# vasil-pashov/sparse_matrix_math

Measured on AMD Instinct MI355X. Metric: CSR SpMV GB/s (% HBM peak) + BiCGStab iters/sec, 10M rows, 1/2/4/8 GPU, higher is better.
Workload: dtype f32

## Files before the change

include/smm_hip.h:

```cpp
#ifndef SMM_HIP_H
#define SMM_HIP_H

#include <stddef.h>

#ifdef __cplusplus
extern "C" {
#endif

#define SMM_HIP_VERSION_MAJOR 0
#define SMM_HIP_VERSION_MINOR 1

#define SMM_HIP_OK 0
#define SMM_HIP_ERR_INVALID (-1)
#define SMM_HIP_ERR_HIP (-2)
#define SMM_HIP_ERR_NO_DEVICE (-3)
#define SMM_HIP_ERR_PRECOND (-4)
#define SMM_HIP_ERR_NOMEM (-5)
#define SMM_HIP_ERR_COMM (-6)

#define SMM_SOLVER_SUCCESS 0
#define SMM_SOLVER_DIVERGED 1
#define SMM_SOLVER_MAX_ITERATIONS_REACHED 2

#define SMM_OP_ASSIGN 0
// ... 22 lines not shown
#define SMM_PATTERN_CONST 3

typedef struct smm_hip_csr smm_hip_csr;
typedef struct smm_hip_precond smm_hip_precond;
typedef void* smm_hip_stream;

int smm_hip_init(int device);
int smm_hip_shutdown(void);
const char* smm_hip_last_error(void);
int smm_hip_uses_std_fma(void);
int smm_hip_device_info(char* name, size_t name_cap, int* cus, size_t* hbm_bytes);
int smm_hip_stream_synchronize(smm_hip_stream stream);

int smm_hip_debug_fail_next_alloc(size_t min_bytes);
int smm_hip_profile_enable(int on);
int smm_hip_profile_read(double* spmv_ms, long long* spmv_launches, int reset);
int smm_hip_profile_read_waits(double* exposed_ms, long long* pairs, int reset);

int smm_hip_csr_create_f32(int rows, int cols, const int* start, const int* positions, const float* values, smm_hip_csr** out);
int smm_hip_csr_create_f64(int rows, int cols, const int* start, const int* positions, const double* values, smm_hip_csr** out);
int smm_hip_csr_create_dev_f32(int rows, int cols, const int* d_start, const int* d_positions, const float* d_values, smm_hip_csr** out);
int smm_hip_csr_create_dev_f64(int rows, int cols, const int* d_start, const int* d_positions, const double* d_values, smm_hip_csr** out);
int smm_hip_csr_destroy(smm_hip_csr* m);
int smm_hip_csr_info(const smm_hip_csr* m, int* rows, int* cols, int* nnz, int* dtype, int* first_active_start);
int smm_hip_csr_set_kernel(smm_hip_csr* m, int family, int lanes_per_row);
int smm_hip_csr_get_kernel(const smm_hip_csr* m, int* family, int* lanes_per_row);
int smm_hip_csr_tile_info(const smm_hip_csr* m, int* tiles, int* tile_nnz_cap, int* tile_max_rows, int* tile_kernel);
int smm_hip_csr_pattern_info(const smm_hip_csr* m, int* encoding, int* offsets);
int smm_hip_csr_kernel_desc(const smm_hip_csr* m, char* name, int name_cap, long long* bytes_per_launch);
int smm_hip_set_march_min_rows(long long const_diagonals_rows, long long values_read_rows);
int smm_hip_set_cg_lazy_x_min_bytes(long long bytes);
int smm_hip_set_cg_fuse_p(int on);
int smm_hip_csr_pattern_allow_const(smm_hip_csr* m, int allow);
int smm_hip_csr_autotune(smm_hip_csr* m);

#define SMM_UPDATE_SET 0
#define SMM_UPDATE_ADD 1
int smm_hip_csr_scale_f32(smm_hip_csr* m, float alpha, smm_hip_stream stream);
int smm_hip_csr_scale_f64(smm_hip_csr* m, double alpha, smm_hip_stream stream);
int smm_hip_csr_axpy_f32(smm_hip_csr* m, float alpha, const smm_hip_csr* other, smm_hip_stream stream);
int smm_hip_csr_axpy_f64(smm_hip_csr* m, double alpha, const smm_hip_csr* other, smm_hip_stream stream);
int smm_hip_csr_zero_f32(smm_hip_csr* m, smm_hip_stream stream);
int smm_hip_csr_zero_f64(smm_hip_csr* m, smm_hip_stream stream);
int smm_hip_csr_update_entries_f32(smm_hip_csr* m, int n, const int* rows, const int* cols, const float* values, int mode, unsigned char* found);
int smm_hip_csr_update_entries_f64(smm_hip_csr* m, int n, const int* rows, const int* cols, const double* values, int mode, unsigned char* found);
int smm_hip_csr_update_entries_dev_f32(smm_hip_csr* m, int n, const int* d_rows, const int* d_cols, const float* d_values, int mode, unsigned char* d_found,
                                       smm_hip_stream stream);
int smm_hip_csr_update_entries_dev_f64(smm_hip_csr* m, int n, const int* d_rows, const int* d_cols, const double* d_values, int mode, unsigned char* d_found,
                                       smm_hip_stream stream);
int smm_hip_csr_set_values_f32(smm_hip_csr* m, const float* values);
int smm_hip_csr_set_values_f64(smm_hip_csr* m, const double* values);
int smm_hip_csr_set_values_dev_f32(smm_hip_csr* m, const float* d_values, smm_hip_stream stream);
int smm_hip_csr_set_values_dev_f64(smm_hip_csr* m, const double* d_values, smm_hip_stream stream);
int smm_hip_csr_get_values_f32(const smm_hip_csr* m, float* values);
int smm_hip_csr_get_values_f64(const smm_hip_csr* m, double* values);
int smm_hip_csr_values_changed_f32(smm_hip_csr* m, smm_hip_stream stream);
int smm_hip_csr_values_changed_f64(smm_hip_csr* m, smm_hip_stream stream);
int smm_hip_csr_same_pattern(const smm_hip_csr* a, const smm_hip_csr* b, int* same);

int smm_hip_spmv_f32(const smm_hip_csr* m, int op, const float* lhs, const float* x, float* out);
int smm_hip_spmv_f64(const smm_hip_csr* m, int op, const double* lhs, const double* x, double* out);
int smm_hip_spmv_dev_f32(const smm_hip_csr* m, int op, const float* d_lhs, const float* d_x, float* d_out, smm_hip_stream stream);
int smm_hip_spmv_dev_f64(const smm_hip_csr* m, int op, const double* d_lhs, const double* d_x, double* d_out, smm_hip_stream stream);

int smm_hip_dot_f32(int n, const float* a, const float* b, float* result);
int smm_hip_dot_f64(int n, const double* a, const double* b, double* result);
// ... 177 lines not shown
```

sparse_matrix_math_amd/_lib.py:

```python
import ctypes
import os
from ctypes import POINTER, c_char_p, c_double, c_float, c_int, c_longlong, c_size_t, c_ulonglong, c_void_p

_HERE = os.path.dirname(os.path.abspath(__file__))

SMM_HIP_OK = 0
SMM_HIP_ERR_INVALID = -1
SMM_HIP_ERR_HIP = -2
SMM_HIP_ERR_NO_DEVICE = -3
SMM_HIP_ERR_PRECOND = -4
SMM_HIP_ERR_NOMEM = -5
SMM_HIP_ERR_COMM = -6


class SmmHipError(RuntimeError):
    def __init__(self, code, message):
        super().__init__(f"libsmm_hip error {code}: {message}")
        self.code = code


def library_path(fma=False):
    if os.environ.get("SMM_HIP_LIBRARY"):
        return os.environ["SMM_HIP_LIBRARY"]
    name = "libsmm_hip_fma.so" if fma else "libsmm_hip.so"
# ... 45 lines not shown
    "smm_hip_csr_update_entries": (c_int, [_P, c_int, _P, _P, _P, c_int, _P]),
    "smm_hip_csr_update_entries_dev": (c_int, [_P, c_int, _P, _P, _P, c_int, _P, _P]),
    "smm_hip_csr_set_values": (c_int, [_P, _P]),
    "smm_hip_csr_set_values_dev": (c_int, [_P, _P, _P]),
    "smm_hip_csr_get_values": (c_int, [_P, _P]),
    "smm_hip_csr_values_changed": (c_int, [_P, _P]),
}



_PLAIN = {
    "smm_hip_init": (c_int, [c_int]),
    "smm_hip_shutdown": (c_int, []),
    "smm_hip_last_error": (c_char_p, []),
    "smm_hip_uses_std_fma": (c_int, []),
    "smm_hip_device_info": (c_int, [c_char_p, c_size_t, POINTER(c_int), POINTER(c_size_t)]),
    "smm_hip_stream_synchronize": (c_int, [_P]),
    "smm_hip_debug_fail_next_alloc": (c_int, [c_size_t]),
    "smm_hip_profile_enable": (c_int, [c_int]),
    "smm_hip_profile_read": (c_int, [POINTER(c_double), POINTER(c_longlong), c_int]),
    "smm_hip_profile_read_waits": (c_int, [POINTER(c_double), POINTER(c_longlong), c_int]),
    "smm_hip_csr_destroy": (c_int, [_P]),
    "smm_hip_csr_info": (c_int, [_P, POINTER(c_int), POINTER(c_int), POINTER(c_int), POINTER(c_int), POINTER(c_int)]),
    "smm_hip_csr_set_kernel": (c_int, [_P, c_int, c_int]),
    "smm_hip_csr_get_kernel": (c_int, [_P, POINTER(c_int), POINTER(c_int)]),
    "smm_hip_csr_autotune": (c_int, [_P]),
    "smm_hip_csr_tile_info": (c_int, [_P, POINTER(c_int), POINTER(c_int), POINTER(c_int), POINTER(c_int)]),
    "smm_hip_csr_pattern_info": (c_int, [_P, POINTER(c_int), POINTER(c_int)]),
    "smm_hip_csr_kernel_desc": (c_int, [_P, c_char_p, c_int, POINTER(c_longlong)]),
    "smm_hip_set_march_min_rows": (c_int, [c_longlong, c_longlong]),
    "smm_hip_set_cg_lazy_x_min_bytes": (c_int, [c_longlong]),
    "smm_hip_set_cg_fuse_p": (c_int, [c_int]),
    "smm_hip_csr_pattern_allow_const": (c_int, [_P, c_int]),
    "smm_hip_csr_same_pattern": (c_int, [_P, _P, POINTER(c_int)]),
    "smm_hip_precond_create": (c_int, [_P, c_int, POINTER(_P)]),
    "smm_hip_precond_create_block": (c_int, [_P, c_int, c_int, POINTER(_P)]),
    "smm_hip_precond_create_block_capped": (c_int, [_P, c_int, c_int, c_int, POINTER(_P)]),
    "smm_hip_precond_block_level_cap": (c_int, [_P, POINTER(c_int)]),
    "smm_hip_precond_create_block_ex": (c_int, [_P, c_int, c_int, c_int, c_int, POINTER(_P)]),
    "smm_hip_precond_block_rows": (c_int, [_P, _P, c_size_t, _P]),
    "smm_hip_precond_block_record_bytes": (c_int, [_P, POINTER(c_int), POINTER(c_int), POINTER(c_int)]),
    "smm_hip_precond_block_count": (c_int, [_P, POINTER(c_int)]),
    "smm_hip_precond_block_bounds": (c_int, [_P, _P, c_size_t]),
    "smm_hip_precond_destroy": (c_int, [_P]),
    "smm_hip_precond_set_sweep": (c_int, [_P, c_int]),
    "smm_hip_precond_take_error": (c_int, [_P, _P]),
    "smm_hip_precond_info": (c_int, [_P, POINTER(c_int), POINTER(c_int), POINTER(c_int)]),
    "smm_hip_gen_poisson2d_nnz": (c_longlong, [c_int, c_int]),
    "smm_hip_gen_stencil3d_nnz": (c_longlong, [c_int, c_int, c_int]),
    "smm_hip_gen_banded_nnz": (c_longlong, [c_int, c_int, c_ulonglong, c_int]),
    "smm_hip_gen_banded_row_start": (c_longlong, [c_int, c_int, c_ulonglong, c_int, c_int]),
    "smm_hip_partials_count": (c_int, []),
    "smm_hip_finish_len": (c_int, []),
    "smm_hip_finish_totals_offset": (c_int, []),
    "smm_hip_cg_resident": (c_int, [c_int]),
    "smm_hip_bicgstab_resident": (c_int, [c_int]),
    "smm_hip_bicgstab_ws_destroy": (c_int, [_P]),
    "smm_hip_cg_ws_status": (c_int, [_P, _P, POINTER(c_int)]),
    "smm_hip_bicgstab_ws_bind": (c_int, [_P, _P, _P, _P]),
    "smm_hip_bicgstab_ws_pointers": (c_int, [_P, POINTER(_P), POINTER(_P), POINTER(_P), POINTER(_P), POINTER(_P), POINTER(_P)]),
    "smm_hip_comm_unique_id": (c_int, [_P]),
    "smm_hip_comm_create_rccl": (c_int, [c_int, c_int, _P, POINTER(_P)]),
    "smm_hip_comm_create_host": (c_int, [c_int, c_int, HOST_ALLREDUCE_FN, HOST_SENDRECV_FN, _P, POINTER(_P)]),
    "smm_hip_comm_create_self": (c_int, [POINTER(_P)]),
    "smm_hip_comm_destroy": (c_int, [_P]),
    "smm_hip_comm_info": (c_int, [_P, POINTER(c_int), POINTER(c_int), POINTER(c_int)]),
# ... 86 lines not shown
```

sparse_matrix_math_amd/csrc/smm_csr_update.hip:

```cpp
#include <algorithm>
#include <cstring>

#include <rocprim/device/device_radix_sort.hpp>

#include "smm_internal.h"

namespace smm {
namespace {

constexpr int UTPB = 256;

typedef float upd_f32x4 __attribute__((ext_vector_type(4)));
typedef double upd_f64x2 __attribute__((ext_vector_type(2)));
template <typename T>
struct Vec16;
template <>
struct Vec16<float> {
	using type = upd_f32x4;
};
template <>
struct Vec16<double> {
	using type = upd_f64x2;
};

// ... 240 lines not shown
}

bool isConstForm(const smm_hip_csr* m) {
	return m->pat_state.load(std::memory_order_acquire) == 1 && m->pat_encoding == 0 && m->pat_const && m->d_pat_cval &&
	       static_cast<int>(m->pat_cval_host.size()) == m->pat_k;
}

template <typename T>
int valuesEdited(smm_hip_csr* m, hipStream_t s, int edit, T alpha, const smm_hip_csr* other) {
	if (m->pat_state.load(std::memory_order_acquire) != 1 || m->pat_encoding != 0) return SMM_HIP_OK;
	std::lock_guard<std::mutex> lock(m->tileMutex);
	if (isConstForm(m)) {
		const int k = m->pat_k;
		std::vector<unsigned long long> bits(m->pat_cval_host);
		bool exact = true;
		if (edit == EDIT_SCALE) {
			for (int j = 0; j < k; ++j) bits[j] = toBits<T>(fromBits<T>(bits[j]) * alpha);
		} else if (edit == EDIT_ZERO) {
			for (int j = 0; j < k; ++j) bits[j] = 0;
		} else if (edit == EDIT_AXPY && other && isConstForm(other) && other->pat_k == k && other->pat_offs_host == m->pat_offs_host) {
			for (int j = 0; j < k; ++j) bits[j] = toBits<T>(fromBits<T>(bits[j]) + alpha * fromBits<T>(other->pat_cval_host[j]));
		} else {
			exact = false;
		}
		if (exact) {
			cvalUpdateKernel<T><<<1, CMAX, 0, s>>>(k, edit == EDIT_SCALE ? 0 : edit == EDIT_AXPY ? 1 : 2, alpha, m->d_pat_cval,
			                                       edit == EDIT_AXPY ? other->d_pat_cval : nullptr);
			SMM_HIP_TRY(hipGetLastError());
			m->pat_cval_host = bits;
		} else {
			SMM_TRY(reverifyConst(m, s));
		}
	}
	return refreshResEll(m, s);
}

int checkHandle(const smm_hip_csr* m, int dtype, const char* what) {
	if (!m) {
		setError("%s: null matrix", what);
		return SMM_HIP_ERR_INVALID;
	}
	if (m->dtype != dtype) {
		setError("%s: the matrix holds the other element type", what);
		return SMM_HIP_ERR_INVALID;
	}
	return ensureInit();
}

template <typename T>
int scaleDev(smm_hip_csr* m, T alpha, hipStream_t s) {
	SMM_TRY(checkHandle(m, dtypeOf<T>(), "csr_scale"));
	SMM_TRY(ensureCsrReady(m, s, true));
	if (m->nnz > 0) {
		T* v = static_cast<T*>(m->d_values);
		if (reinterpret_cast<uintptr_t>(v) % 16 == 0) valuesUpdateKernel<T, false, true><<<gridFor(m->nnz / (16 / sizeof(T)) + 1), UTPB, 0, s>>>(m->nnz, alpha, v, nullptr);
		else valuesUpdateKernel<T, false, false><<<gridFor(m->nnz), UTPB, 0, s>>>(m->nnz, alpha, v, nullptr);
		SMM_HIP_TRY(hipGetLastError());
	}
	return valuesEdited<T>(m, s, EDIT_SCALE, alpha, nullptr);
}

template <typename T>
int axpyDev(smm_hip_csr* m, T alpha, const smm_hip_csr* other, hipStream_t s) {
	SMM_TRY(checkHandle(m, dtypeOf<T>(), "csr_axpy"));
	SMM_TRY(checkHandle(other, dtypeOf<T>(), "csr_axpy"));
	bool same = false;
// ... 180 lines not shown
```

sparse_matrix_math_amd/csrc/smm_internal.h:

```cpp
#pragma once
#include <hip/hip_runtime.h>

#include <cstddef>
#include <cstdint>
#include <cstdio>
#include <atomic>
#include <chrono>
#include <cstdlib>
#include <cstring>
#include <mutex>
#include <string>
#include <type_traits>
#include <vector>

#include "../../include/smm_hip.h"

namespace smm {

void setError(const char* fmt, ...);
int hipFail(hipError_t e, const char* what, const char* file, int line);

#define SMM_HIP_TRY(expr)                                             \
	do {                                                              \
		hipError_t _e = (expr);                                       \
// ... 87 lines not shown
}

struct smm_hip_csr {
	int rows = 0, cols = 0, nnz = 0, dtype = 0;
	int firstActiveStart = 0;
	bool ready = false;
	bool kernelForced = false;
	std::mutex readyMutex;
	int* d_start = nullptr;
	int* d_positions = nullptr;
	void* d_values = nullptr;
	bool owns = false;
	std::atomic<int> kernelWord{SMM_SPMV_VECTOR | (4 << 8)};
	int family() const { return kernelWord.load(std::memory_order_acquire) & 0xFF; }
	int lanes() const { return kernelWord.load(std::memory_order_acquire) >> 8; }
	void setKernel(int family, int lanes) { kernelWord.store((family & 0xFF) | (lanes << 8), std::memory_order_release); }
	std::mutex adoptMutex;
	int* d_rowblocks = nullptr;
	int n_rowblocks = 0;
	int stream_nnz_cap = 0;
	int stream_max_rows = 0;
	int stream_chunk_tiles = 0;
	int stream_mid_len = 0;
	int max_row_len = -1;
	std::mutex tileMutex;
	std::atomic<int> pat_state{0};
	int pat_encoding = 0;
	unsigned short* d_pat_codes = nullptr;
	bool pat_const = false;
	unsigned long long* d_pat_cval = nullptr;
	std::vector<unsigned long long> pat_cval_host;
	void* d_res_ell = nullptr;
	bool pat_const_off = false;
	int pat_max_off = 0;
	bool march_ok = false;
	int march_P = 0, march_H = 0, march_lo = 0, march_hi = 0;
	bool march_clusters = false;
	unsigned* d_pat_masks32 = nullptr;
	unsigned char* d_pat_masks8 = nullptr;
	std::vector<int> pat_offs_host;
	int pat_k = 0;
	int* d_pat_off = nullptr;
	unsigned long long* d_pat_masks = nullptr;
	int* d_pat_rowblocks = nullptr;
	int pat_n_rowblocks = 0;
	int pat_nnz_cap = 0;
	int pat_max_rows = 0;
	int pat_chunk_tiles = 0;
	int split_tile_max[3] = {-1, -1, -1};
	bool split_uneven = false;
	std::atomic<unsigned long long> uid{0};
	std::mutex editMutex;
	std::vector<std::pair<unsigned long long, bool>> patternSeen;
};

struct smm_hip_precond {
	int kind = SMM_PRECOND_NONE;
	int dtype = 0;
	const smm_hip_csr* a = nullptr;
	void* d_values = nullptr;
	size_t n_values = 0;
	int* d_order_lo = nullptr;
	int* d_order_up = nullptr;
	std::vector<int> lvl_ptr_lo, lvl_ptr_up;
	struct smm_precond_plan* plan = nullptr;
	struct smm_precond_block* blk = nullptr;
// ... 16 lines not shown
constexpr int SPMV_FINISH = 0x200;
constexpr int SPMV_LEAVE_ROOM = 0x400;
constexpr int SPMV_DIV_LHS = 0x800;
constexpr int SPMV_OP_DIV = 3;
constexpr int SPMV_ADD_DIV = 0x1000;
constexpr int SPMV_OP_ADD_DIV = 4;
constexpr int SPMV_HALF_TILES = 0x2000;
constexpr int SPMV_NO_FULL_ROWS = 0x4000;
constexpr int PARTS_TOTALS = 2 * NPART;
constexpr int PARTS_TICKETS = 16;
constexpr int PARTS_LEN = 2 * NPART + 2 + 2 * (PARTS_TICKETS + 1);
template <typename T>
__host__ __device__ inline unsigned* partsTicket(T* partials) { return reinterpret_cast<unsigned*>(partials + PARTS_TOTALS + 2); }
inline int spmvOutFlags(const smm_hip_csr* m, size_t elemBytes) {
	static const int forced = [] {
		const char* env = getenv("SMM_HIP_NT_OUT");
		return env ? atoi(env) : -1;
	}();
	if (forced >= 0) return forced ? SPMV_NT_OUT : 0;
	return static_cast<double>(m->rows) * static_cast<double>(elemBytes) >= 64.0 * 1024 * 1024 ? SPMV_NT_OUT : 0;
}

int buildRowBlocks(smm_hip_csr* m, int capNnz, int maxRows, hipStream_t s);
int buildTileTable(const smm_hip_csr* m, int capNnz, int maxRows, hipStream_t s, int** blocks, int* nBlocks, int* chunkTiles);
int cutRows(const int* d_start, int rows, long long nnz, int capNnz, int maxRows, hipStream_t s, int2** tiles, int* nTiles, int tilesPerChunk = 0);
int ensureCsrReady(const smm_hip_csr* m, hipStream_t s, bool streamKnown);
int ensurePattern(smm_hip_csr* m, hipStream_t s = nullptr, bool streamKnown = false, bool quiet = false, bool masksOnly = false);
int adoptPatternForSolver(const smm_hip_csr* m, int plannedIterations, hipStream_t s);
void adoptPatternQuietly(const smm_hip_csr* m, hipStream_t s);
int patternLanesFor(const smm_hip_csr* m);
const char* patternKernelDesc(const smm_hip_csr* m, int lanes, long long* bytes);
void planMarch(smm_hip_csr* m);
int refreshResEll(smm_hip_csr* a, hipStream_t s);
int marchBuildMasks32(smm_hip_csr* m, hipStream_t s);
template <typename K>
inline int occupancyCached(std::atomic<long long>& slot, K kernel, int tpb, size_t lds, int fallback) {
	const long long seen = slot.load(std::memory_order_acquire);
	if (seen != 0 && static_cast<size_t>(seen >> 8) == lds) return static_cast<int>(seen & 0xFF);
	int n = 0;
	if (hipOccupancyMaxActiveBlocksPerMultiprocessor(&n, kernel, tpb, lds) != hipSuccess || n < 1) {
		(void)hipGetLastError();
		n = fallback;
	}
	n = n > 255 ? 255 : n;
	slot.store((static_cast<long long>(lds) << 8) | n, std::memory_order_release);
	return n;
}
template <typename K>
inline bool ensureDynamicLds(std::atomic<int>& granted, K kernel, size_t lds) {
	if (lds <= 64 * 1024) return true;
	int have = granted.load(std::memory_order_acquire);
	while (static_cast<size_t>(have) < lds) {
		if (hipFuncSetAttribute(reinterpret_cast<const void*>(kernel), hipFuncAttributeMaxDynamicSharedMemorySize, static_cast<int>(lds)) != hipSuccess) {
			(void)hipGetLastError();
			return false;
		}
		if (granted.compare_exchange_weak(have, static_cast<int>(lds), std::memory_order_acq_rel)) break;
	}
	return true;
}
inline int forcedWgsPerCU() {
	static const int forced = [] {
		const char* env = getenv("SMM_HIP_STREAM_WGS_PER_CU");
		return env ? (atoi(env) > 1 ? atoi(env) : 1) : 0;
	}();
	return forced;
}

bool cgHalfTiles(const smm_hip_csr* m, size_t elemBytes);
long long cgLazyMinBytes();
bool updateNT(long long n, size_t elemBytes, int vectors);
bool masksMarchApplies(const smm_hip_csr* m);
bool constMarchApplies(const smm_hip_csr* m);
template <typename T>
bool launchPatMasksMarch(const smm_hip_csr* m, int op, const T* lhs, const T* divisor, const T* x, T* out, int dotMode, const T* w1, T* partials,
                         const int* doneFlag, hipStream_t s);
template <typename T>
bool launchPatConstMarch(const smm_hip_csr* m, int op, const T* lhs, const T* divisor, const T* x, T* out, int dotMode, const T* w1, T* partials,
                         const int* doneFlag, hipStream_t s);
template <typename T>
int launchSpmvPattern(const smm_hip_csr* m, int lanes, int op, const T* lhs, const T* divisor, const T* x, T* out, int dotMode, const T* w1, T* partials,
                      const int* doneFlag, hipStream_t s);
void chooseSpmvConfig(smm_hip_csr* m);
template <typename T>
int launchSpmvSplit(const smm_hip_csr* aLoc, const smm_hip_csr* aRem, int op, const T* lhs, const T* divisor, const T* own, const T* ext, T* out, int dotMode,
                    const T* w1, T* partials, const int* doneFlag, int extraFlags, const unsigned long long* landed, unsigned long long seq, unsigned long long* err,
                    long long ticks, hipStream_t s, const struct P2PSlotArgs* slots = nullptr, int sumsLdsMax = 16384, unsigned long long* waited = nullptr);
void launchSplitSignal(unsigned long long* landed, unsigned long long seq, hipStream_t s);
void preloadSplitUnit();
template <typename T>
struct CgFuseBook {
	const int* pad = nullptr;
	T* rrPing = nullptr;
	T* res = nullptr;
	int *iters = nullptr, *done = nullptr, *status = nullptr, *flushIter = nullptr;
};
template <typename T>
struct CgFuseArgs {
	const T* r;
	T* pNew;
	CgFuseBook<T> bk;
	const T* partsC;
	T eps;
	int par, iter;
	const T* totalsC = nullptr;
	int extraFlags = 0;
};
bool constMarchFusable(const smm_hip_csr* m, size_t elemBytes);
template <typename T>
bool launchConstMarchFusedP(const smm_hip_csr* m, const T* pOld, T* Ap, T* partials, const int* doneFlag, const CgFuseArgs<T>& f, hipStream_t s);

template <typename T>
// ... 100 lines not shown
```

sparse_matrix_math_amd/csrc/smm_runtime.hip:

```cpp
#include <atomic>
#include <cstdarg>
#include <chrono>
#include <map>
#include <thread>

#include "smm_internal.h"

namespace smm {

static thread_local std::string g_lastError;
static std::mutex g_mutex;
static bool g_inited = false;
static int g_device = -1;
static int g_cus = 0;
static hipStream_t g_stream = nullptr;

void setError(const char* fmt, ...) {
	char buf[1024];
	va_list ap;
	va_start(ap, fmt);
	vsnprintf(buf, sizeof(buf), fmt, ap);
	va_end(ap);
	g_lastError = buf;
}
// ... 657 lines not shown
	}
	if (exposed_ms) *exposed_ms = total;
	if (pairs) *pairs = static_cast<long long>(g_profWaitUsed);
	if (reset) g_profWaitUsed = 0;
	return SMM_HIP_OK;
}

int smm_hip_csr_create_f32(int rows, int cols, const int* start, const int* positions, const float* values, smm_hip_csr** out) {
	return csrCreate<float>(rows, cols, start, positions, values, false, out);
}
int smm_hip_csr_create_f64(int rows, int cols, const int* start, const int* positions, const double* values, smm_hip_csr** out) {
	return csrCreate<double>(rows, cols, start, positions, values, false, out);
}
int smm_hip_csr_create_dev_f32(int rows, int cols, const int* d_start, const int* d_positions, const float* d_values, smm_hip_csr** out) {
	return csrCreate<float>(rows, cols, d_start, d_positions, d_values, true, out);
}
int smm_hip_csr_create_dev_f64(int rows, int cols, const int* d_start, const int* d_positions, const double* d_values, smm_hip_csr** out) {
	return csrCreate<double>(rows, cols, d_start, d_positions, d_values, true, out);
}

int smm_hip_csr_destroy(smm_hip_csr* m) {
	if (!m) return SMM_HIP_OK;
	if (m->owns) {
		devFree(m->d_start);
		devFree(m->d_positions);
		devFree(m->d_values);
	}
	devFree(m->d_rowblocks);
	devFree(m->d_pat_off);
	devFree(m->d_pat_masks);
	devFree(m->d_pat_codes);
	devFree(m->d_pat_cval);
	devFree(m->d_res_ell);
	devFree(m->d_pat_masks32);
	devFree(m->d_pat_masks8);
	devFree(m->d_pat_rowblocks);
	delete m;
	return SMM_HIP_OK;
}

int smm_hip_csr_info(const smm_hip_csr* m, int* rows, int* cols, int* nnz, int* dtype, int* first_active_start) {
	if (!m) {
		setError("csr_info: null handle");
		return SMM_HIP_ERR_INVALID;
	}
	if (nnz || first_active_start) SMM_TRY(ensureCsrReady(m, nullptr, false));
	if (rows) *rows = m->rows;
	if (cols) *cols = m->cols;
	if (nnz) *nnz = m->nnz;
	if (dtype) *dtype = m->dtype;
	if (first_active_start) *first_active_start = m->firstActiveStart;
	return SMM_HIP_OK;
}

}
```

sparse_matrix_math_amd/csrc/smm_spmv_pattern.hip:

```cpp
#include <algorithm>
#include <cmath>

#include <rocprim/device/device_radix_sort.hpp>

#include "smm_device.h"
#include "smm_internal.h"
#include "smm_pattern_dev.h"

namespace smm {

__global__ __launch_bounds__(TPB) void patBuildMasks(int rows, const int* __restrict__ meta, const int* __restrict__ offs, const int* __restrict__ start,
                                                     const int* __restrict__ positions, unsigned long long* __restrict__ masks,
                                                     int* __restrict__ flags, const void* __restrict__ values, int elemBytes,
                                                     const unsigned long long* __restrict__ cvalBits) {
	if (meta[1] != 0) return;
	const int k = meta[0];
	if (values != nullptr && k > 32) values = nullptr;
	int* mismatch = flags;
	__shared__ int sOff[MAXOFF];
	__shared__ unsigned long long sCval[MAXOFF];
	const bool checkConst = values != nullptr && flags[1] == 0;
	if (checkConst && threadIdx.x < k) sCval[threadIdx.x] = cvalBits[threadIdx.x];
	bool varies = false;
	__shared__ int sRow[TPB / WAVE][WAVE + 1];
// ... 1462 lines not shown
	const int L = std::min(lanes, WAVE);
	if (m->pat_encoding == 1) {
		*bytes = nnz * (s + 2) + startBytes + vectors;
		return "spmvDictKernel";
	}
	if (L == 1 && m->pat_const && !m->pat_const_off) {
		static const bool marchOn = [] {
			const char* env = getenv("SMM_HIP_CONST_MARCH");
			return env ? atoi(env) != 0 : true;
		}();
		const bool march = marchOn && constMarchApplies(m);
		const bool bytesMasks = march && !m->march_clusters && m->d_pat_masks8 && m->pat_k - m->march_lo - m->march_hi == 5;
		*bytes = rows * (bytesMasks ? 1 : march ? 4 : 8) + vectors;
		return march ? (m->march_clusters ? "spmvPatternConstMarch3Kernel" : "spmvPatternConstMarchKernel") : "spmvPatternConstKernel";
	}
	*bytes = nnz * s + rows * 8 + startBytes + vectors;
	if (L == 1 && masksMarchApplies(m)) {
		static const bool masksMarchOn = [] {
			const char* env = getenv("SMM_HIP_MASKS_MARCH");
			return env ? atoi(env) != 0 : true;
		}();
		if (masksMarchOn) {
			*bytes = nnz * s + rows + (rows / 64 + 1) * 4 + vectors;
			return "spmvPatternMasksMarchKernel";
		}
	}
	if (L == 1) {
		static const int waveEnv = [] {
			const char* env = getenv("SMM_HIP_PATTERN_WAVE");
			return env ? atoi(env) : -1;
		}();
		if (waveEnv != 0 && m->pat_k <= 16) return "spmvPatternWaveKernel";
	}
	if ((L == 2 || L == 4) && patUseTile(L)) return "spmvPatternTileKernel";
	return "spmvPatternKernel";
}

static bool patNeedsTiles(const smm_hip_csr* m, int L) {
	if (L != 1 || m->pat_encoding != 0) return true;
	if (m->pat_const && !m->pat_const_off) return false;
	static const int waveEnv = [] {
		const char* env = getenv("SMM_HIP_PATTERN_WAVE");
		return env ? atoi(env) : -1;
	}();
	return !(waveEnv != 0 && m->pat_k <= 16);
}

static int buildPatternTiles(smm_hip_csr* m, int capNnz, int maxRows, hipStream_t s) {
	int* blocks = nullptr;
	int n = 0, chunk = 0;
	SMM_TRY(buildTileTable(m, capNnz, maxRows, s, &blocks, &n, &chunk));
	devFree(m->d_pat_rowblocks);
	m->d_pat_rowblocks = blocks;
	m->pat_n_rowblocks = n;
	m->pat_nnz_cap = capNnz;
	m->pat_max_rows = maxRows;
	m->pat_chunk_tiles = chunk;
	return SMM_HIP_OK;
}

template <typename T>
int launchSpmvPattern(const smm_hip_csr* m, int lanes, int op, const T* lhs, const T* divisor, const T* x, T* out, int dotMode, const T* w1, T* partials,
                      const int* doneFlag, hipStream_t s) {
	auto* mm = const_cast<smm_hip_csr*>(m);
	SMM_TRY(ensurePattern(mm, s, true));
	const int L = std::min(lanes, WAVE);
	const int capNnz = patCap<T>(m, L) - 3;
	const int maxRows = TPB / L;
	if (patNeedsTiles(m, L)) {
		std::lock_guard<std::mutex> lock(mm->tileMutex);
		if (!m->d_pat_rowblocks || m->pat_nnz_cap != capNnz || m->pat_max_rows != maxRows) {
			SetupTrace trace("pattern: tile table");
			SMM_TRY(buildPatternTiles(mm, capNnz, maxRows, s));
		}
	}
	switch (L) {
	case 1: launchPat<T, 1>(m, op, lhs, divisor, x, out, dotMode, w1, partials, doneFlag, s); break;
	case 2: launchPat<T, 2>(m, op, lhs, divisor, x, out, dotMode, w1, partials, doneFlag, s); break;
	case 4: launchPat<T, 4>(m, op, lhs, divisor, x, out, dotMode, w1, partials, doneFlag, s); break;
	default: launchPat<T, 8>(m, op, lhs, divisor, x, out, dotMode, w1, partials, doneFlag, s); break;
	}
	SMM_HIP_TRY(hipGetLastError());
	return SMM_HIP_OK;
}

template int launchSpmvPattern<float>(const smm_hip_csr*, int, int, const float*, const float*, const float*, float*, int, const float*, float*, const int*, hipStream_t);
template int launchSpmvPattern<double>(const smm_hip_csr*, int, int, const double*, const double*, const double*, double*, int, const double*, double*, const int*, hipStream_t);

}

extern "C" int smm_hip_csr_pattern_allow_const(smm_hip_csr* m, int allow) {
	if (!m) {
		smm::setError("csr_pattern_allow_const: null matrix");
		return SMM_HIP_ERR_INVALID;
	}
	m->pat_const_off = allow == 0;
	return SMM_HIP_OK;
}

extern "C" int smm_hip_csr_pattern_info(const smm_hip_csr* m, int* encoding, int* offsets) {
	if (!m) {
		smm::setError("csr_pattern_info: null matrix");
		return SMM_HIP_ERR_INVALID;
	}
	if (encoding) *encoding = m->pat_state > 0 ? (m->pat_encoding == 1 ? SMM_PATTERN_CODES : m->pat_const && !m->pat_const_off ? SMM_PATTERN_CONST : SMM_PATTERN_MASKS) : SMM_PATTERN_NONE;
	if (offsets) *offsets = m->pat_state > 0 ? m->pat_k : 0;
	return SMM_HIP_OK;
// ... 2 lines not shown
```

sparse_matrix_math_amd/host.py:

```python
import ctypes
import enum

import numpy as np

from . import _lib
from ._lib import check


class SolverStatus(enum.IntEnum):
    SUCCESS = 0
    DIVERGED = 1
    MAX_ITERATIONS_REACHED = 2


class SolverPreconditioner(enum.IntEnum):
    NONE = 0
    JACOBI = 1
    ILU0 = 2
    SYMMETRIC_GAUS_SEIDEL = 3
    IC0 = 4
    BLOCK_ILU0 = 5
    BLOCK_SGS = 6


# ... 232 lines not shown
        check(fn(self._h, op, plhs, _host(mult, self.dtype, "mult", self.cols), _host(out, self.dtype, "out", self.rows, True)))

    def rMult(self, mult, res):
        self._spmv(OP_ASSIGN, None, mult, res)

    def rMultAdd(self, lhs, mult, out):
        self._spmv(OP_ADD, lhs, mult, out)

    def rMultSub(self, lhs, mult, out):
        self._spmv(OP_SUB, lhs, mult, out)

    def spmv_dev(self, op, d_lhs, d_x, d_out, stream=None):
        check(_fn("smm_hip_spmv_dev", self._suf)(self._h, int(op), _dptr(d_lhs), _dptr(d_x), _dptr(d_out), _dptr(stream)))

    def tile_info(self):
        v = [ctypes.c_int() for _ in range(4)]
        check(_lib.load().smm_hip_csr_tile_info(self._h, *[ctypes.byref(c) for c in v]))
        return tuple(c.value for c in v)

    def pattern_info(self):
        enc, k = ctypes.c_int(), ctypes.c_int()
        check(_lib.load().smm_hip_csr_pattern_info(self._h, ctypes.byref(enc), ctypes.byref(k)))
        return enc.value, k.value

    def kernel_desc(self):
        buf = ctypes.create_string_buffer(64)
        nbytes = ctypes.c_longlong()
        check(_lib.load().smm_hip_csr_kernel_desc(self._h, buf, 64, ctypes.byref(nbytes)))
        return buf.value.decode(), nbytes.value

    def pattern_allow_const(self, allow):
        check(_lib.load().smm_hip_csr_pattern_allow_const(self._h, 1 if allow else 0))

    def _edited(self, stream):
        if stream is None:
            synchronize(None)

    def scale(self, alpha, stream=None):
        check(_fn("smm_hip_csr_scale", self._suf)(self._h, float(alpha), _dptr(stream)))
        self._edited(stream)

    def axpy(self, alpha, other, stream=None):
        check(_fn("smm_hip_csr_axpy", self._suf)(self._h, float(alpha), other._h, _dptr(stream)))
        self._edited(stream)

    def zero(self, stream=None):
        check(_fn("smm_hip_csr_zero", self._suf)(self._h, _dptr(stream)))
        self._edited(stream)

    def __imul__(self, alpha):
        self.scale(alpha)
        return self

    def inplaceAdd(self, other):
        self.axpy(1.0, other)

    def inplaceSubtract(self, other):
        self.axpy(-1.0, other)

    def zeroValues(self):
        self.zero()

    def hasSameNonZeroPattern(self, other):
        same = ctypes.c_int()
        check(_lib.load().smm_hip_csr_same_pattern(self._h, other._h, ctypes.byref(same)))
        return bool(same.value)
# ... 176 lines not shown
```

Baseline: 902.7.

## Add wave-interleaved slot copy of CSR values for uniform-pattern SpMV

```diff
diff --git a/include/smm_hip.h b/include/smm_hip.h
--- a/include/smm_hip.h
+++ b/include/smm_hip.h
@@ -78,6 +78,7 @@
 int smm_hip_set_cg_lazy_x_min_bytes(long long bytes);
 int smm_hip_set_cg_fuse_p(int on);
 int smm_hip_csr_pattern_allow_const(smm_hip_csr* m, int allow);
+int smm_hip_csr_pattern_slots(smm_hip_csr* m, int mode);
 int smm_hip_csr_autotune(smm_hip_csr* m);
 
 #define SMM_UPDATE_SET 0
diff --git a/sparse_matrix_math_amd/_lib.py b/sparse_matrix_math_amd/_lib.py
--- a/sparse_matrix_math_amd/_lib.py
+++ b/sparse_matrix_math_amd/_lib.py
@@ -101,6 +101,7 @@
     "smm_hip_set_cg_lazy_x_min_bytes": (c_int, [c_longlong]),
     "smm_hip_set_cg_fuse_p": (c_int, [c_int]),
     "smm_hip_csr_pattern_allow_const": (c_int, [_P, c_int]),
+    "smm_hip_csr_pattern_slots": (c_int, [_P, c_int]),
     "smm_hip_csr_same_pattern": (c_int, [_P, _P, POINTER(c_int)]),
     "smm_hip_precond_create": (c_int, [_P, c_int, POINTER(_P)]),
     "smm_hip_precond_create_block": (c_int, [_P, c_int, c_int, POINTER(_P)]),
diff --git a/sparse_matrix_math_amd/csrc/smm_csr_update.hip b/sparse_matrix_math_amd/csrc/smm_csr_update.hip
--- a/sparse_matrix_math_amd/csrc/smm_csr_update.hip
+++ b/sparse_matrix_math_amd/csrc/smm_csr_update.hip
@@ -296,6 +296,7 @@
 			SMM_TRY(reverifyConst(m, s));
 		}
 	}
+	SMM_TRY(refreshPatternSlots(m, s));
 	return refreshResEll(m, s);
 }
 
diff --git a/sparse_matrix_math_amd/csrc/smm_internal.h b/sparse_matrix_math_amd/csrc/smm_internal.h
--- a/sparse_matrix_math_amd/csrc/smm_internal.h
+++ b/sparse_matrix_math_amd/csrc/smm_internal.h
@@ -143,6 +143,12 @@
 	std::vector<unsigned long long> pat_cval_host;
 	void* d_res_ell = nullptr;
 	bool pat_const_off = false;
+	void* d_pat_slots = nullptr;
+	long long* d_pat_slot_base = nullptr;
+	int pat_slots_state = 0;
+	int pat_slots_mode = -1;
+	long long pat_slots_elems = 0;
+	int pat_slots_waves = 0, pat_slots_uniform = 0;
 	int pat_max_off = 0;
 	bool march_ok = false;
 	int march_P = 0, march_H = 0, march_lo = 0, march_hi = 0;
@@ -225,6 +231,10 @@
 const char* patternKernelDesc(const smm_hip_csr* m, int lanes, long long* bytes);
 void planMarch(smm_hip_csr* m);
 int refreshResEll(smm_hip_csr* a, hipStream_t s);
+bool ensurePatternSlots(smm_hip_csr* m, int lanes, hipStream_t s);
+bool patternSlotsChosen(const smm_hip_csr* m, int lanes);
+long long patternSlotsBytes(const smm_hip_csr* m);
+int refreshPatternSlots(smm_hip_csr* m, hipStream_t s);
 int marchBuildMasks32(smm_hip_csr* m, hipStream_t s);
 template <typename K>
 inline int occupancyCached(std::atomic<long long>& slot, K kernel, int tpb, size_t lds, int fallback) {
@@ -271,6 +281,9 @@
 template <typename T>
 bool launchPatConstMarch(const smm_hip_csr* m, int op, const T* lhs, const T* divisor, const T* x, T* out, int dotMode, const T* w1, T* partials,
                          const int* doneFlag, hipStream_t s);
+template <typename T>
+void launchPatSlots(const smm_hip_csr* m, int lanes, int op, const T* lhs, const T* divisor, const T* x, T* out, int dotMode, const T* w1, T* partials,
+                    const int* doneFlag, hipStream_t s);
 template <typename T>
 int launchSpmvPattern(const smm_hip_csr* m, int lanes, int op, const T* lhs, const T* divisor, const T* x, T* out, int dotMode, const T* w1, T* partials,
                       const int* doneFlag, hipStream_t s);
diff --git a/sparse_matrix_math_amd/csrc/smm_runtime.hip b/sparse_matrix_math_amd/csrc/smm_runtime.hip
--- a/sparse_matrix_math_amd/csrc/smm_runtime.hip
+++ b/sparse_matrix_math_amd/csrc/smm_runtime.hip
@@ -713,6 +713,8 @@
 	devFree(m->d_pat_codes);
 	devFree(m->d_pat_cval);
 	devFree(m->d_res_ell);
+	devFree(m->d_pat_slots);
+	devFree(m->d_pat_slot_base);
 	devFree(m->d_pat_masks32);
 	devFree(m->d_pat_masks8);
 	devFree(m->d_pat_rowblocks);
diff --git a/sparse_matrix_math_amd/csrc/smm_spmv_pattern.hip b/sparse_matrix_math_amd/csrc/smm_spmv_pattern.hip
--- a/sparse_matrix_math_amd/csrc/smm_spmv_pattern.hip
+++ b/sparse_matrix_math_amd/csrc/smm_spmv_pattern.hip
@@ -1518,7 +1518,13 @@
 		}();
 		if (waveEnv != 0 && m->pat_k <= 16) return "spmvPatternWaveKernel";
 	}
-	if ((L == 2 || L == 4) && patUseTile(L)) return "spmvPatternTileKernel";
+	if ((L == 2 || L == 4) && patUseTile(L)) {
+		if (patternSlotsChosen(m, L)) {
+			*bytes = patternSlotsBytes(m);
+			return "spmvPatternSlotsKernel";
+		}
+		return "spmvPatternTileKernel";
+	}
 	return "spmvPatternKernel";
 }
 
@@ -1553,12 +1559,19 @@
 	const int L = std::min(lanes, WAVE);
 	const int capNnz = patCap<T>(m, L) - 3;
 	const int maxRows = TPB / L;
+	bool slots = false;
 	if (patNeedsTiles(m, L)) {
 		std::lock_guard<std::mutex> lock(mm->tileMutex);
 		if (!m->d_pat_rowblocks || m->pat_nnz_cap != capNnz || m->pat_max_rows != maxRows) {
 			SetupTrace trace("pattern: tile table");
 			SMM_TRY(buildPatternTiles(mm, capNnz, maxRows, s));
 		}
+		slots = ensurePatternSlots(mm, L, s);
+	}
+	if (slots) {
+		launchPatSlots<T>(m, L, op, lhs, divisor, x, out, dotMode, w1, partials, doneFlag, s);
+		SMM_HIP_TRY(hipGetLastError());
+		return SMM_HIP_OK;
 	}
 	switch (L) {
 	case 1: launchPat<T, 1>(m, op, lhs, divisor, x, out, dotMode, w1, partials, doneFlag, s); break;
diff --git a/sparse_matrix_math_amd/csrc/smm_spmv_slots.hip b/sparse_matrix_math_amd/csrc/smm_spmv_slots.hip
--- /dev/null
+++ b/sparse_matrix_math_amd/csrc/smm_spmv_slots.hip
@@ -0,0 +1,318 @@
+#include <algorithm>
+
+#include <rocprim/device/device_scan.hpp>
+
+#include "smm_pattern_dev.h"
+
+namespace smm {
+
+constexpr int SLOT_WAVES = TPB / WAVE;
+
+__global__ __launch_bounds__(TPB) void slotsCountKernel(int rows, int nWaves, const unsigned long long* __restrict__ masks, long long* __restrict__ counts,
+                                                        int* __restrict__ uniformWaves) {
+	const int lane = threadIdx.x & (WAVE - 1);
+	int mine = 0;
+	for (int w = (blockIdx.x * TPB + threadIdx.x) / WAVE; w < nWaves; w += gridDim.x * SLOT_WAVES) {
+		const int row = w * WAVE + lane;
+		const unsigned long long mm = row < rows ? masks[row] : ~0ULL;
+		const unsigned long long lead = patUniform64(mm);
+		const bool uniform = lead != 0ULL && __builtin_amdgcn_ballot_w64(!(row < rows && mm == lead)) == 0ULL;
+		if (lane == 0) {
+			counts[w] = uniform ? static_cast<long long>(__builtin_popcountll(lead)) * WAVE : 0;
+			mine += uniform;
+		}
+	}
+	if (lane == 0 && mine) atomicAdd(uniformWaves, mine);
+}
+
+__global__ __launch_bounds__(TPB) void slotsMarkKernel(int nWaves, const long long* __restrict__ counts, long long* __restrict__ base) {
+	for (int w = blockIdx.x * TPB + threadIdx.x; w < nWaves; w += gridDim.x * TPB) {
+		if (counts[w] == 0) base[w] = -1;
+	}
+}
+
+template <typename T>
+__global__ __launch_bounds__(TPB) void slotsFillKernel(int nWaves, const long long* __restrict__ base, const unsigned long long* __restrict__ masks,
+                                                       const int* __restrict__ start, const T* __restrict__ values, T* __restrict__ slots) {
+	const int lane = threadIdx.x & (WAVE - 1);
+	for (int w = (blockIdx.x * TPB + threadIdx.x) / WAVE; w < nWaves; w += gridDim.x * SLOT_WAVES) {
+		const long long b = base[w];
+		if (b < 0) continue;
+		const int row = w * WAVE + lane;
+		const int len = __builtin_popcountll(masks[w * WAVE]);
+		const T* src = values + start[row];
+		T* dst = slots + b + lane;
+		for (int e = 0; e < len; ++e) dst[static_cast<long long>(e) * WAVE] = src[e];
+	}
+}
+
+template <typename T, int L, int G>
+__global__ __launch_bounds__(TPB) void spmvPatternSlotsKernel(int rows, int nWaves, int chunkWaves, const int* __restrict__ offs,
+                                                              const long long* __restrict__ base, const unsigned long long* __restrict__ masks,
+                                                              const T* __restrict__ slots, const int* __restrict__ start, const int* __restrict__ positions,
+                                                              const T* __restrict__ values, int opFlags, const T* lhs, const T* __restrict__ divisor,
+                                                              const T* __restrict__ x, T* out, int dotMode, const T* __restrict__ w1,
+                                                              T* __restrict__ partials, const int* __restrict__ doneFlag) {
+	static_assert(L == 2 || L == 4, "pieces per row");
+	__shared__ T red[4];
+	if (doneFlag && *doneFlag) return;
+	const int op = opFlags & 0xFF;
+	const bool ntOut = (opFlags & SPMV_NT_OUT) != 0;
+	const int t = threadIdx.x;
+	const int lane = t & (WAVE - 1);
+	const int wave = __builtin_amdgcn_readfirstlane(t >> 6);
+	const int nGroups = min(8, static_cast<int>(gridDim.x));
+	const int xcdGroup = blockIdx.x % nGroups;
+	const int groupSlots = (static_cast<int>(gridDim.x) - xcdGroup + nGroups - 1) / nGroups;
+	const int wEnd = min(nWaves, (xcdGroup + 1) * chunkWaves);
+	T acc0 = T(0), acc1 = T(0);
+	for (int w = xcdGroup * chunkWaves + static_cast<int>(blockIdx.x / nGroups) * SLOT_WAVES + wave; w < wEnd; w += groupSlots * SLOT_WAVES) {
+		const int row = w * WAVE + lane;
+		const long long b = base[w];
+		T dot = T(0);
+		if (b >= 0) {
+			const unsigned long long lead = masks[w * WAVE];
+			const int len = __builtin_popcountll(lead);
+			const int pl = (len + L - 1) / L;
+			const int offLane = offs[lane < len ? selectBit(lead, lane) : 0];
+			const T* const xr = x + row;
+			const T* const sv = slots + b + lane;
+			T part[L];
+#pragma unroll
+			for (int q = 0; q < L; ++q) part[q] = T(0);
+			for (int i = 0; i < pl; i += G) {
+				T vv[L][G], xv[L][G];
+#pragma unroll
+				for (int q = 0; q < L; ++q) {
+#pragma unroll
+					for (int u = 0; u < G; ++u) {
+						const int e = min(q * pl + i + u, len - 1);
+						vv[q][u] = __builtin_nontemporal_load(sv + static_cast<long long>(e) * WAVE);
+						xv[q][u] = xr[__builtin_amdgcn_readlane(offLane, e)];
+					}
+				}
+#pragma unroll
+				for (int q = 0; q < L; ++q) {
+#pragma unroll
+					for (int u = 0; u < G; ++u) {
+						if (i + u < pl && q * pl + i + u < len) part[q] = smmFma(vv[q][u], xv[q][u], part[q]);
+					}
+				}
+			}
+			dot = part[0];
+#pragma unroll
+			for (int q = 1; q < L; ++q) dot += part[q];
+		} else if (row < rows) {
+			dot = patRowDirect<T, L>(start[row], start[row + 1], values, positions, x);
+		}
+		if (row < rows) {
+			const T o = patApplyOp(op, lhs, divisor, row, dot);
+			storeOut(out + row, o, ntOut);
+			if (dotMode == 2) acc0 += o * o;
+			if (dotMode) acc1 += o * w1[row];
+		}
+	}
+	if (dotMode) {
+		if (dotMode == 2) {
+			const T s0 = blockSum256(acc0, red);
+			if (t == 0) partials[blockIdx.x] = s0;
+		}
+		const T s1 = blockSum256(acc1, red);
+		if (t == 0) partials[(dotMode == 2 ? NPART : 0) + blockIdx.x] = s1;
+		for (int i = gridDim.x + blockIdx.x * TPB + t; i < NPART; i += gridDim.x * TPB) {
+			partials[i] = T(0);
+			if (dotMode == 2) partials[NPART + i] = T(0);
+		}
+		if (opFlags & SPMV_FINISH) lastBlockSums<T>(partials, NPART, dotMode == 2 ? 2 : 1, partials + PARTS_TOTALS, partsTicket(partials));
+	}
+}
+
+static int slotsEnvMode() {
+	static const int mode = [] {
+		const char* env = getenv("SMM_HIP_PATTERN_SLOTS");
+		return env ? (atoi(env) != 0 ? 1 : 0) : -1;
+	}();
+	return mode;
+}
+
+static int slotsMode(const smm_hip_csr* m) { return m->pat_slots_mode >= 0 ? m->pat_slots_mode : slotsEnvMode(); }
+
+static bool slotsApplies(const smm_hip_csr* m, int lanes) {
+	if (lanes != 2 && lanes != 4) return false;
+	if (m->pat_encoding != 0 || (m->pat_const && !m->pat_const_off)) return false;
+	static const bool fullRows = [] {
+		const char* env = getenv("SMM_HIP_FULL_ROWS");
+		const char* variant = getenv("SMM_HIP_PATTERN_VARIANT");
+		return !(env && atoi(env) == 0) && !(variant && atoi(variant) == 0);
+	}();
+	return fullRows;
+}
+
+static bool slotsWanted(const smm_hip_csr* m, int lanes, bool* forced) {
+	const int mode = slotsMode(m);
+	*forced = mode == 1;
+	if (mode == 0 || !slotsApplies(m, lanes)) return false;
+	return mode == 1 || mode == 2 || !m->kernelForced;
+}
+
+static bool slotsUniformEnough(const smm_hip_csr* m) {
+	return static_cast<long long>(m->pat_slots_uniform) * 100 >= static_cast<long long>(m->pat_slots_waves) * 99;
+}
+
+bool patternSlotsChosen(const smm_hip_csr* m, int lanes) {
+	bool forced = false;
+	if (!slotsWanted(m, lanes, &forced) || m->pat_slots_state != 1 || !m->d_pat_slots) return false;
+	return forced || slotsUniformEnough(m);
+}
+
+template <typename T>
+static int slotsFill(smm_hip_csr* m, hipStream_t s) {
+	const int nWaves = m->pat_slots_waves;
+	const int grid = std::max(1, std::min(4096, (nWaves + SLOT_WAVES - 1) / SLOT_WAVES));
+	slotsFillKernel<T><<<grid, TPB, 0, s>>>(nWaves, m->d_pat_slot_base, m->d_pat_masks, m->d_start, static_cast<const T*>(m->d_values),
+	                                         static_cast<T*>(m->d_pat_slots));
+	SMM_HIP_TRY(hipGetLastError());
+	return SMM_HIP_OK;
+}
+
+template <typename T>
+static int slotsBuild(smm_hip_csr* m, bool forced, hipStream_t s) {
+	SetupTrace trace("pattern: slots copy");
+	const int nWaves = (m->rows + WAVE - 1) / WAVE;
+	DevBuf<long long> counts, base;
+	DevBuf<int> uniform;
+	DevBuf<unsigned char> temp;
+	SMM_TRY(counts.alloc(nWaves));
+	SMM_TRY(base.alloc(static_cast<size_t>(nWaves) + 1));
+	SMM_TRY(uniform.alloc(1));
+	SMM_HIP_TRY(hipMemsetAsync(uniform.p, 0, sizeof(int), s));
+	SMM_HIP_TRY(hipMemsetAsync(base.p, 0, sizeof(long long), s));
+	const int grid = std::max(1, std::min(4096, (nWaves + SLOT_WAVES - 1) / SLOT_WAVES));
+	slotsCountKernel<<<grid, TPB, 0, s>>>(m->rows, nWaves, m->d_pat_masks, counts.p, uniform.p);
+	SMM_HIP_TRY(hipGetLastError());
+	size_t tempBytes = 0;
+	SMM_HIP_TRY(rocprim::inclusive_scan(nullptr, tempBytes, counts.p, base.p + 1, static_cast<size_t>(nWaves), rocprim::plus<long long>(), s));
+	SMM_TRY(temp.alloc(tempBytes ? tempBytes : 1));
+	SMM_HIP_TRY(rocprim::inclusive_scan(temp.p, tempBytes, counts.p, base.p + 1, static_cast<size_t>(nWaves), rocprim::plus<long long>(), s));
+	slotsMarkKernel<<<std::max(1, std::min(4096, (nWaves + TPB - 1) / TPB)), TPB, 0, s>>>(nWaves, counts.p, base.p);
+	SMM_HIP_TRY(hipGetLastError());
+	long long total = 0;
+	int nUniform = 0;
+	SMM_HIP_TRY(hipMemcpyAsync(&total, base.p + nWaves, sizeof(total), hipMemcpyDeviceToHost, s));
+	SMM_HIP_TRY(hipMemcpyAsync(&nUniform, uniform.p, sizeof(nUniform), hipMemcpyDeviceToHost, s));
+	SMM_HIP_TRY(hipStreamSynchronize(s));
+	m->pat_slots_waves = nWaves;
+	m->pat_slots_uniform = nUniform;
+	m->pat_slots_elems = total;
+	if (!forced && !slotsUniformEnough(m)) return SMM_HIP_ERR_INVALID;
+	const size_t bytes = static_cast<size_t>(std::max(1LL, total)) * sizeof(T);
+	size_t freeB = 0, totalB = 0;
+	SMM_HIP_TRY(hipMemGetInfo(&freeB, &totalB));
+	if (freeB < bytes + std::max<size_t>(size_t(1) << 30, totalB / 16)) return SMM_HIP_ERR_INVALID;
+	void* p = nullptr;
+	SMM_TRY(devAlloc(&p, bytes));
+	m->d_pat_slots = p;
+	m->d_pat_slot_base = base.detach();
+	int st = slotsFill<T>(m, s);
+	hipError_t e = st == SMM_HIP_OK ? hipStreamSynchronize(s) : hipSuccess;
+	if (st != SMM_HIP_OK || e != hipSuccess) {
+		devFree(m->d_pat_slots);
+		devFree(m->d_pat_slot_base);
+		m->d_pat_slots = nullptr;
+		m->d_pat_slot_base = nullptr;
+		return st != SMM_HIP_OK ? st : hipFail(e, "slotsFillKernel", __FILE__, __LINE__);
+	}
+	return SMM_HIP_OK;
+}
+
+bool ensurePatternSlots(smm_hip_csr* m, int lanes, hipStream_t s) {
+	bool forced = false;
+	if (!slotsWanted(m, lanes, &forced)) return false;
+	if (m->pat_slots_state == 1 && m->d_pat_slots) return forced || slotsUniformEnough(m);
+	if (m->pat_slots_state < 0 && !forced) return false;
+	const int st = m->dtype == SMM_DTYPE_F32 ? slotsBuild<float>(m, forced, s) : slotsBuild<double>(m, forced, s);
+	if (st != SMM_HIP_OK) {
+		m->pat_slots_state = -1;
+		(void)hipGetLastError();
+		setError("");
+		return false;
+	}
+	m->pat_slots_state = 1;
+	return true;
+}
+
+int refreshPatternSlots(smm_hip_csr* m, hipStream_t s) {
+	if (!m->d_pat_slots || !m->d_pat_slot_base || m->rows <= 0) return SMM_HIP_OK;
+	return m->dtype == SMM_DTYPE_F32 ? slotsFill<float>(m, s) : slotsFill<double>(m, s);
+}
+
+long long patternSlotsBytes(const smm_hip_csr* m) {
+	const long long s = m->dtype == SMM_DTYPE_F32 ? 4 : 8;
+	const long long rows = m->rows, nnz = m->nnz;
+	const long long otherRows = std::max(0LL, rows - 64LL * m->pat_slots_uniform);
+	const long long otherNnz = std::max(0LL, nnz - m->pat_slots_elems);
+	return m->pat_slots_elems * s + static_cast<long long>(m->pat_slots_waves) * 16 + otherNnz * (s + 4) + (otherRows + m->pat_slots_waves) * 4 +
+	       static_cast<long long>(m->cols) * s + rows * s;
+}
+
+static int slotsBatch(const smm_hip_csr* m, int lanes) {
+	const long long len = m->pat_slots_uniform > 0 ? (m->pat_slots_elems + 32LL * m->pat_slots_uniform) / (64LL * m->pat_slots_uniform) : 1;
+	const int p = static_cast<int>(std::max(1LL, (len + lanes - 1) / lanes));
+	const int nb = (p + 15) / 16;
+	const int g = (p + nb - 1) / nb;
+	return g <= 8 ? 8 : g <= 13 ? 13 : 16;
+}
+
+template <typename T, int L, int G>
+static void launchSlotsG(const smm_hip_csr* m, int op, const T* lhs, const T* divisor, const T* x, T* out, int dotMode, const T* w1, T* partials,
+                         const int* doneFlag, hipStream_t s) {
+	static std::atomic<long long> occ{0};
+	const int perCU = occupancyCached(occ, spmvPatternSlotsKernel<T, L, G>, TPB, 0, 4);
+	const int cus = (op & SPMV_LEAVE_ROOM) ? std::max(8, numCUs() - 8) : numCUs();
+	const int nWaves = m->pat_slots_waves;
+	const int grid = std::max(1, std::min(std::min((nWaves + SLOT_WAVES - 1) / SLOT_WAVES, cus * perCU), NPART));
+	const int nGroups = std::min(8, grid);
+	const int chunkWaves = (nWaves + nGroups - 1) / nGroups;
+	spmvPatternSlotsKernel<T, L, G><<<grid, TPB, 0, s>>>(m->rows, nWaves, chunkWaves, m->d_pat_off, m->d_pat_slot_base, m->d_pat_masks,
+	                                                    static_cast<const T*>(m->d_pat_slots), m->d_start, m->d_positions, static_cast<const T*>(m->d_values),
+	                                                    (op & ~SPMV_LEAVE_ROOM) | spmvOutFlags(m, sizeof(T)), lhs, divisor, x, out, dotMode, w1, partials,
+	                                                    doneFlag);
+}
+
+template <typename T, int L>
+static void launchSlotsL(const smm_hip_csr* m, int op, const T* lhs, const T* divisor, const T* x, T* out, int dotMode, const T* w1, T* partials,
+                         const int* doneFlag, hipStream_t s) {
+	switch (slotsBatch(m, L)) {
+	case 8: launchSlotsG<T, L, 8>(m, op, lhs, divisor, x, out, dotMode, w1, partials, doneFlag, s); break;
+	case 13: launchSlotsG<T, L, 13>(m, op, lhs, divisor, x, out, dotMode, w1, partials, doneFlag, s); break;
+	default: launchSlotsG<T, L, 16>(m, op, lhs, divisor, x, out, dotMode, w1, partials, doneFlag, s); break;
+	}
+}
+
+template <typename T>
+void launchPatSlots(const smm_hip_csr* m, int lanes, int op, const T* lhs, const T* divisor, const T* x, T* out, int dotMode, const T* w1, T* partials,
+                    const int* doneFlag, hipStream_t s) {
+	if (lanes == 2) {
+		launchSlotsL<T, 2>(m, op, lhs, divisor, x, out, dotMode, w1, partials, doneFlag, s);
+	} else {
+		launchSlotsL<T, 4>(m, op, lhs, divisor, x, out, dotMode, w1, partials, doneFlag, s);
+	}
+}
+
+template void launchPatSlots<float>(const smm_hip_csr*, int, int, const float*, const float*, const float*, float*, int, const float*, float*, const int*,
+                                    hipStream_t);
+template void launchPatSlots<double>(const smm_hip_csr*, int, int, const double*, const double*, const double*, double*, int, const double*, double*,
+                                     const int*, hipStream_t);
+
+}
+
+extern "C" int smm_hip_csr_pattern_slots(smm_hip_csr* m, int mode) {
+	if (!m || mode < -1 || mode > 2) {
+		smm::setError("csr_pattern_slots: null matrix or a mode other than -1, 0, 1, 2");
+		return SMM_HIP_ERR_INVALID;
+	}
+	std::lock_guard<std::mutex> lock(m->tileMutex);
+	m->pat_slots_mode = mode;
+	if (mode == 1 && m->pat_slots_state < 0) m->pat_slots_state = 0;
+	return SMM_HIP_OK;
+}
diff --git a/sparse_matrix_math_amd/host.py b/sparse_matrix_math_amd/host.py
--- a/sparse_matrix_math_amd/host.py
+++ b/sparse_matrix_math_amd/host.py
@@ -288,6 +288,9 @@
     def pattern_allow_const(self, allow):
         check(_lib.load().smm_hip_csr_pattern_allow_const(self._h, 1 if allow else 0))
 
+    def pattern_slots(self, mode):
+        check(_lib.load().smm_hip_csr_pattern_slots(self._h, int(mode)))
+
     def _edited(self, stream):
         if stream is None:
             synchronize(None)
```

After: 936.4 (median of 6 runs). 1.04x the previous value.
